# jojolebarjos/board-game-simulator-python

Measured on AMD Instinct MI355X. Metric: env-steps/sec, Connect4(6,7,4) random rollout, batch=2^20 per GPU, higher is better.
Workload: dtype u64

## Files before the change

### board-game-simulator-python_amd/csrc/bgs_host.hip

```cpp
#include <immintrin.h>
#include <limits.h>
#include <linux/futex.h>
#include <pthread.h>
#include <sched.h>
#include <sys/syscall.h>
#include <time.h>
#include <unistd.h>

#include <atomic>
#include <chrono>
#include <condition_variable>
#include <cstdlib>
#include <cstdio>
#include <algorithm>
#include <cstring>
#include <mutex>
#include <new>
#include <thread>
#include <vector>

#include "bgs_capi_util.h"
#include "bgs_common.h"
#include "bgs_internal.h"

struct bgs_event {
    int device;
    hipEvent_t ev;
};

namespace {

using bgs::fail;

struct ExpandTable {
    uint64_t pairs[256];
    ExpandTable() {
        for (int byte = 0; byte < 256; ++byte) {
            uint64_t four = 0;
            for (int j = 0; j < 4; ++j) four |= (uint64_t)bgs::reward_pair((uint32_t)(byte >> (2 * j)) & 3u) << (16 * j);
            pairs[byte] = four;
        }
    }
};
const ExpandTable g_expand;

template <bool STREAM>
__attribute__((target("avx2"))) int64_t expand_avx2(const uint8_t* src, int64_t code_bytes, int8_t* dst) {
    const __m256i spread = _mm256_setr_epi8(0, 0, 0, 0, 1, 1, 1, 1, 2, 2, 2, 2, 3, 3, 3, 3,
                                            4, 4, 4, 4, 5, 5, 5, 5, 6, 6, 6, 6, 7, 7, 7, 7);
    const __m256i field = _mm256_set1_epi32((int)0xC0300C03u);
    const __m256i one = _mm256_set1_epi32(0x40100401);
    const __m256i two = _mm256_set1_epi32((int)0x80200802u);
    int64_t i = 0;
    for (; i + 8 <= code_bytes; i += 8) {
        long long eight;
        memcpy(&eight, src + i, 8);
        const __m256i rep = _mm256_shuffle_epi8(_mm256_set1_epi64x(eight), spread);
        const __m256i f = _mm256_and_si256(rep, field);
        const __m256i is1 = _mm256_cmpeq_epi8(f, one), is2 = _mm256_cmpeq_epi8(f, two);
        const __m256i r0 = _mm256_sub_epi8(is2, is1), r1 = _mm256_sub_epi8(is1, is2);
        const __m256i lo = _mm256_unpacklo_epi8(r0, r1), hi = _mm256_unpackhi_epi8(r0, r1);
        const __m256i first = _mm256_permute2x128_si256(lo, hi, 0x20), second = _mm256_permute2x128_si256(lo, hi, 0x31);
        if (STREAM) {
            _mm256_stream_si256(reinterpret_cast<__m256i*>(dst + 8 * i), first);
            _mm256_stream_si256(reinterpret_cast<__m256i*>(dst + 8 * i + 32), second);
        } else {
            _mm256_storeu_si256(reinterpret_cast<__m256i*>(dst + 8 * i), first);
            _mm256_storeu_si256(reinterpret_cast<__m256i*>(dst + 8 * i + 32), second);
        }
    }
    if (STREAM) _mm_sfence();
    return i;
}

const bool g_have_avx2 = __builtin_cpu_supports("avx2");
const bool g_stream_stores = bgs::experiment("no_stream_stores") == nullptr;

void expand_range(const uint8_t* packed, int64_t first, int64_t count, int8_t* reward) {
    const int64_t whole = count / 4;
    const uint8_t* src = packed + first / 4;
    int8_t* out = reward + 2 * first;
    int64_t i0 = 0;
    if (g_have_avx2) {
        const bool stream = (reinterpret_cast<uintptr_t>(out) & 31u) == 0 && whole >= (1 << 14) && g_stream_stores;
        i0 = stream ? expand_avx2<true>(src, whole, out) : expand_avx2<false>(src, whole, out);
    }
    for (int64_t i = i0; i < whole; ++i) memcpy(out + 8 * i, &g_expand.pairs[src[i]], 8);
    for (int64_t g = first + whole * 4; g < first + count; ++g) {
        const uint16_t pair = bgs::reward_pair((uint32_t)(packed[g / 4] >> (2 * (g & 3))) & 3u);
        memcpy(reward + 2 * g, &pair, 2);
    }
}

struct CellFormat {
    int cells = 0;
    int nwc = 0;
    int sets = 0;
    int offset = 0;
    int weight[4] = {0, 0, 0, 0};
};

struct SpreadTable {
    uint64_t v[256];
    SpreadTable() {
        for (int byte = 0; byte < 256; ++byte) {
            uint64_t w = 0;
            for (int b = 0; b < 8; ++b) w |= (uint64_t)((byte >> b) & 1) << (8 * b);
            v[byte] = w;
        }
    }
};
const SpreadTable g_spread;

__attribute__((target("avx512f,avx512bw"))) void expand_cells_avx512(const uint64_t* wire, int64_t n, const CellFormat& f,
                                                                      int64_t first, int64_t count, int8_t* out) {
    const __m512i base = _mm512_set1_epi8((char)f.offset);
    __m512i weight[4];
    for (int p = 0; p < f.sets; ++p) weight[p] = _mm512_set1_epi8((char)f.weight[p]);
    alignas(64) int8_t block[64 * 256 + 64];
    const bool lines = f.cells <= 256 && g_stream_stores && (reinterpret_cast<uintptr_t>(out) & 63u) == 0;
#define BGS_ONE_GAME(i_)                                                                                              \
    do {                                                                                                                \
        int8_t* dst_ = out + (i_)*f.cells;                                                                              \
        for (int j = 0; j < f.nwc; ++j) {                                                                               \
            __m512i acc = base;                                                                                         \
// ... 95 lines not shown
    const bool have = fgets(list, sizeof list, f) != nullptr;
    fclose(f);
    if (!have) return false;
    cpu_set_t allowed;
    if (sched_getaffinity(0, sizeof allowed, &allowed) != 0) return false;
    int any = 0;
    char* save = nullptr;
    for (char* tok = strtok_r(list, ",\n", &save); tok; tok = strtok_r(nullptr, ",\n", &save)) {
        int lo = 0, hi = 0;
        const int k = sscanf(tok, "%d-%d", &lo, &hi);
        if (k < 1) continue;
        if (k == 1) hi = lo;
        for (int c = lo; c <= hi && c < CPU_SETSIZE; ++c)
            if (CPU_ISSET(c, &allowed)) {
                CPU_SET(c, out);
                ++any;
            }
    }
    return any > 0;
}

}

namespace {
inline bool sink_trace_on() {
    static const bool on = bgs::experiment("sink_trace") != nullptr;
    return on;
}
inline double mono_us() {
    return std::chrono::duration<double, std::micro>(std::chrono::steady_clock::now().time_since_epoch()).count();
}
}

static bool codes_hold_a_zero(const uint8_t* codes, int64_t first, int64_t count) {
    const uint8_t* p = codes + first / 4;
    const int64_t whole = count / 4;
    int64_t i = 0;
    uint64_t seen = 0;
    for (; i + 8 <= whole; i += 8) {
        uint64_t x;
        memcpy(&x, p + i, 8);
        seen |= ~(x | (x >> 1)) & 0x5555555555555555ull;
    }
    for (; i < whole; ++i) seen |= (uint64_t)(~(p[i] | (p[i] >> 1)) & 0x55u);
    for (int64_t k = 0; k < count - whole * 4; ++k) seen |= ((p[whole] >> (2 * k)) & 3u) == 0u ? 1u : 0u;
    return seen != 0;
}

struct bgs_reward_sink {
    int device = 0;
    int64_t max_games = 0;
    int slots = 0;
    int ring = 0;
    int threads = 0;
    std::vector<uint8_t*> pinned;
    std::vector<uint8_t*> mapped;
    std::vector<hipEvent_t> landed;
    bool grids = false;
    CellFormat cells;
    size_t slot_bytes = 0;
    struct Job {
        int64_t n_games = 0;
        int8_t* host_reward = nullptr;
        int event_slot = 0;
        bool all_end = false;
    };
    std::vector<Job> jobs;
    std::mutex mu;
    std::condition_variable cv_submit;
    std::condition_variable cv_landed;
    std::condition_variable cv_done;
    int64_t claimed = 0;
    int64_t submitted = 0;
    volatile int64_t* progress = nullptr;
    int64_t landed_upto = 0;
    int64_t completed = 0;
    std::vector<int> parts_done;
    std::vector<char> slot_ok;
    bool stop = false;
    std::vector<int64_t> failed_tickets;
    bool poll = false;
    std::vector<std::thread> workers;
    std::atomic<int64_t> a_submitted{0}, a_landed{0}, a_completed{0};
    std::atomic<bool> a_stop{false};
    std::atomic<int> urgent{0};
    int spin_us = 0;
    int wait_spin_us = 200;

    bool spin_for(const std::atomic<int64_t>& counter, int64_t ticket) const {
        if (counter.load(std::memory_order_acquire) > ticket) return true;
        if (spin_us <= 0) return false;
        const auto until = std::chrono::steady_clock::now() + std::chrono::microseconds(spin_us);
        for (;;) {
            for (int i = 0; i < 64; ++i) {
                if (counter.load(std::memory_order_acquire) > ticket || a_stop.load(std::memory_order_relaxed)) return true;
                _mm_pause();
            }
            if (std::chrono::steady_clock::now() >= until) return false;
        }
    }

    void work(int t) {
        (void)hipSetDevice(device);
        for (int64_t ticket = 0;; ++ticket) {
            const int slot = (int)(ticket % ring);
            Job job;
            bool ok = true;
            if (t == 0) {
                spin_for(a_submitted, ticket);
                {
                    std::unique_lock<std::mutex> lock(mu);
                    cv_submit.wait(lock, [&] { return stop || submitted > ticket; });
                    if (submitted <= ticket) return;
                    job = jobs[slot];
                }
                if (job.n_games == 0) {
                    ok = false;
                } else if (poll || urgent.load(std::memory_order_relaxed) > 0) {
                    hipError_t e;
                    while ((e = hipEventQuery(landed[job.event_slot])) == hipErrorNotReady) _mm_pause();
                    ok = e == hipSuccess;
                } else {
                    ok = hipEventSynchronize(landed[job.event_slot]) == hipSuccess;
                }
                if (sink_trace_on()) fprintf(stderr, "sink-trace ticket %lld landed %.1f\n", (long long)ticket, mono_us());
                {
                    std::lock_guard<std::mutex> lock(mu);
                    if (!ok && job.n_games != 0) failed_tickets.push_back(ticket);
                    slot_ok[slot] = ok;
                    landed_upto = ticket + 1;
                    a_landed.store(ticket + 1, std::memory_order_release);
                }
                cv_landed.notify_all();
            } else {
                if (urgent.load(std::memory_order_relaxed) > 0) {
                    const auto until = std::chrono::steady_clock::now() + std::chrono::microseconds(2000);
                    while (a_landed.load(std::memory_order_acquire) <= ticket && !a_stop.load(std::memory_order_relaxed) &&
                           urgent.load(std::memory_order_relaxed) > 0 && std::chrono::steady_clock::now() < until)
                        for (int i = 0; i < 16; ++i) _mm_pause();
                } else {
                    spin_for(a_landed, ticket);
                }
                std::unique_lock<std::mutex> lock(mu);
                cv_landed.wait(lock, [&] { return stop || landed_upto > ticket; });
                if (landed_upto <= ticket) return;
                job = jobs[slot];
                ok = slot_ok[slot];
            }
            const int expanders = threads > 1 ? threads - 1 : 1;
            const int share = threads > 1 ? t - 1 : 0;
            if (threads > 1 && t == 0) continue;
            const double trace_t0 = sink_trace_on() ? mono_us() : 0.0;
            if (ok && grids) {
                const int64_t blocks = (job.n_games + 63) / 64;
                const int64_t g0 = blocks * share / expanders * 64;
                const int64_t g1 = share + 1 == expanders ? job.n_games : blocks * (share + 1) / expanders * 64;
                static const bool skip = bgs::experiment("grid_no_expand") != nullptr;
                if (g1 > g0 && !skip) expand_cells(pinned[slot], job.n_games, cells, g0, g1 - g0, job.host_reward);
            } else if (ok) {
                const int64_t bytes = (job.n_games + 3) / 4;
                const int64_t b0 = bytes * share / expanders, b1 = bytes * (share + 1) / expanders;
                const int64_t first = b0 * 4;
                int64_t count = b1 * 4 - first;
                if (first + count > job.n_games) count = job.n_games - first;
                if (count > 0) expand_range(pinned[slot], first, count, job.host_reward);
                if (count > 0 && job.all_end && codes_hold_a_zero(pinned[slot], first, count)) {
                    std::lock_guard<std::mutex> lock(mu);
                    if (std::find(failed_tickets.begin(), failed_tickets.end(), ticket) == failed_tickets.end()) failed_tickets.push_back(ticket);
                }
            }
            if (sink_trace_on()) fprintf(stderr, "sink-trace ticket %lld worker %d expand %.1f .. %.1f\n", (long long)ticket, t, trace_t0, mono_us());
            {
                std::lock_guard<std::mutex> lock(mu);
                if (++parts_done[slot] == expanders) {
                    parts_done[slot] = 0;
                    ++completed;
                    a_completed.store(completed, std::memory_order_release);
                    cv_done.notify_all();
                    if (progress) progress_store_max(progress, completed);
                }
            }
        }
    }
};

namespace {

int64_t claim(bgs_reward_sink* s, bool ahead = false) {
    const int bound = ahead ? s->ring : s->slots;
    s->spin_for(s->a_completed, s->a_submitted.load(std::memory_order_relaxed) - bound);
    std::unique_lock<std::mutex> lock(s->mu);
    s->cv_done.wait(lock, [&] { return s->claimed - s->completed < bound; });
    return s->claimed++;
}

void publish(bgs_reward_sink* s, int64_t ticket, int64_t n_games, int8_t* host_reward, bool ok = true, int64_t event_ticket = -1,
             bool all_end = false) {
    {
        std::unique_lock<std::mutex> lock(s->mu);
// ... 147 lines not shown
    const hipError_t err = hipEventQuery(e->ev);
    if (err == hipSuccess) *done = 1;
    else if (err == hipErrorNotReady) *done = 0;
    else return fail(BGS_ERR_RUNTIME, "hipEventQuery failed: %s", hipGetErrorString(err));
    return BGS_OK;
}

int bgs_read_reward_async(bgs_batch* b, int8_t* host_dst, bgs_event* done) {
    NEED(b != nullptr && host_dst != nullptr, "NULL argument");
    int rc = enter_device(b->device);
    if (rc) return rc;
    HIP_TRY(hipMemcpyAsync(host_dst, b->d_reward, (size_t)b->n * 2, hipMemcpyDeviceToHost, b->stream));
    if (done) HIP_TRY(hipEventRecord(done->ev, b->stream));
    return BGS_OK;
}

int bgs_read_outcomes_async(bgs_batch* b, uint8_t* host_dst, bgs_event* done) {
    NEED(b != nullptr && host_dst != nullptr, "NULL argument");
    int rc = enter_device(b->device);
    if (rc) return rc;
    const size_t bytes = (size_t)(b->n + 3) / 4;
    NEED(bytes <= b->staging_bytes, "staging buffer too small");
    uint8_t* d_packed = b->d_staging;
    bgs::pack_outcomes(b, d_packed);
    HIP_TRY(hipGetLastError());
    HIP_TRY(hipMemcpyAsync(host_dst, d_packed, bytes, hipMemcpyDeviceToHost, b->stream));
    if (done) HIP_TRY(hipEventRecord(done->ev, b->stream));
    return BGS_OK;
}

int bgs_expand_outcomes_host(const uint8_t* packed, int64_t first, int64_t count, int8_t* reward) {
    NEED(packed != nullptr && reward != nullptr, "NULL argument");
    NEED(first >= 0 && count >= 0 && (first & 3) == 0, "first must be a non-negative multiple of 4, count >= 0");
    expand_range(packed, first, count, reward);
    return BGS_OK;
}

int bgs_rollout_to_host(bgs_batch* b, uint64_t seed, int32_t max_plies, uint32_t flags, void* host_dst, int codes,
                        bgs_event* done) {
    int rc = bgs_rollout(b, seed, max_plies, flags);
    if (rc) return rc;
    return codes ? bgs_read_outcomes_async(b, static_cast<uint8_t*>(host_dst), done)
                 : bgs_read_reward_async(b, static_cast<int8_t*>(host_dst), done);
}

static int make_sink(int device, int64_t max_games, int slots, int threads, size_t slot_bytes, const CellFormat* cells,
                     bgs_reward_sink** out) {
    NEED(out != nullptr, "out is NULL");
    *out = nullptr;
    NEED(max_games >= 1 && slots >= 1 && slots <= 256 && threads >= 1 && threads <= 256,
         "need max_games >= 1, 1 <= slots <= 256, 1 <= threads <= 256");
    int rc = enter_device(device);
    if (rc) return rc;
    bgs_reward_sink* s = new (std::nothrow) bgs_reward_sink();
    NEED(s != nullptr, "out of host memory");
    s->device = device;
    s->max_games = max_games;
    s->slot_bytes = slot_bytes;
    if (cells) {
        s->grids = true;
        s->cells = *cells;
    }
    s->slots = slots;
    s->ring = cells ? slots : std::max(slots, bgs::kSinkGroupRing);
    const int ring = s->ring;
    s->threads = threads;
    s->jobs.resize(ring);
    if (const char* env = bgs::experiment("sink_poll")) s->poll = atoi(env) != 0;
    if (const char* env = bgs::experiment("sink_wait_spin_us")) {
        const int v = atoi(env);
        if (v >= 0 && v <= 1000000) s->wait_spin_us = v;
    }
    if (const char* env = bgs::experiment("sink_spin_us")) {
        const int v = atoi(env);
        if (v >= 0 && v <= 1000000) s->spin_us = v;
    }
    s->parts_done.assign(ring, 0);
    s->slot_ok.assign(ring, 1);
    const size_t bytes = slot_bytes;
    hipError_t err = hipSuccess;
    const char* aff0 = getenv("BGS_SINK_AFFINITY");
    const bool place = !(aff0 && atoi(aff0) == 0);
    cpu_set_t node_cpus, caller_cpus;
    const bool moved = place && device_node_cpus(device, &node_cpus) && sched_getaffinity(0, sizeof caller_cpus, &caller_cpus) == 0 &&
                       sched_setaffinity(0, sizeof node_cpus, &node_cpus) == 0;
    for (int k = 0; k < ring && err == hipSuccess; ++k) {
        void* host = nullptr;
        void* dev = nullptr;
        hipEvent_t ev = nullptr;
        err = hipHostMalloc(&host, bytes, hipHostMallocMapped);
        if (err == hipSuccess) s->pinned.push_back(static_cast<uint8_t*>(host));
        if (err == hipSuccess) err = hipHostGetDevicePointer(&dev, host, 0);
        if (err == hipSuccess) s->mapped.push_back(static_cast<uint8_t*>(dev));
        if (err == hipSuccess) err = hipEventCreateWithFlags(&ev, hipEventDisableTiming);
        if (err == hipSuccess) s->landed.push_back(ev);
    }
    if (moved) (void)sched_setaffinity(0, sizeof caller_cpus, &caller_cpus);
// ... 254 lines not shown
```

### board-game-simulator-python_amd/csrc/connect_kernels.hip

```cpp
#include <type_traits>

#include "bgs_common.h"
#include "bgs_internal.h"
#include "connect_board.h"

#ifndef BGS_TU_ID
#define BGS_TU_ID "unknown"
#endif
extern "C" const char bgs_tu_id_connect[] = BGS_TU_ID;

namespace bgs {
namespace {

template <int NW_, int SH, int SW, int SK>
struct Geo {
    static constexpr int NW = NW_;
    static constexpr int STATIC_H = SH, STATIC_W = SW, STATIC_K = SK;
    static constexpr int MAXW = SW ? SW : BGS_CONNECT_MAX_W;
    int rh, rw, rk;
    __device__ __forceinline__ int h() const { return SH ? SH : rh; }
    __device__ __forceinline__ int w() const { return SW ? SW : rw; }
    __device__ __forceinline__ int k() const { return SK ? SK : rk; }
    __device__ __forceinline__ uint32_t all_columns() const { return (1u << w()) - 1u; }
};
// ... 632 lines not shown
            uint64_t carry;
            asm("v_mad_u64_u32 %0, %1, %2, %3, %4" : "=v"(cmp64), "=s"(carry) : "v"(idx - op), "s"(ONES), "v"(eights));
        }
        const uint32_t cmp = (uint32_t)cmp64;
        uint32_t col = (uint32_t)__popc(cmp & column_top);
        if (g.w() >= 8) col &= 7u;
        const uint32_t sh = col * 4u;
        const uint32_t v = (h4 >> sh) & 15u;
        uint32_t base = col * stride + top;
        asm("" : "+v"(base));
        uint32_t pos = base - v;
        if ((uint32_t)g.w() * stride + top > 63u) pos &= 63u;
        const uint64_t bit = 1ull << pos;
        mine = ((uint64_t)and_or((uint32_t)(bit >> 32), act, (uint32_t)(mine >> 32)) << 32) |
               and_or((uint32_t)bit, act, (uint32_t)mine);
        h4 += act << sh;
        op = (h4 >> 3) & ONES;
        if (g.k() == 4) return ply_run_of_four(g, mine, pos);
        Bits<1> b;
        b.w[0] = mine;
        return has_run(g, b);
    }
    template <uint32_t J>
    __device__ __forceinline__ void full(const G& g, uint32_t draw, uint64_t (&q)[2], uint32_t& h4, uint32_t& op,
                                         uint32_t& alive, bool& won_any) const {
        const bool won = drop(g, draw, alive, q[J & 1u], h4, op);
        won_any = won_any || won;
        alive = (won || op == 0u) ? 0u : alive;
    }
    __device__ __forceinline__ void cheap(const G& g, uint32_t j, uint32_t draw, uint64_t (&q)[2], uint32_t& h4) const {
        const uint32_t col = sample_index(draw, (uint32_t)g.w());
        const uint32_t sh = col * 4u;
        const uint32_t v = (h4 >> sh) & 15u;
        const uint32_t pos = col * stride + top - v;
        q[j & 1u] |= 1ull << pos;
        h4 -= 1u << sh;
    }
    __device__ __forceinline__ static uint32_t outcome_of(const uint64_t (&q)[2], bool won_any) {
        const uint32_t stones = (uint32_t)__popcll(q[0]) + (uint32_t)__popcll(q[1]);
        return connect_outcome_byte(stones, won_any);
    }
};

template <class G, bool CAPPED, bool FROM_INITIAL, bool CODES, bool PER_PLY>
__global__ void __launch_bounds__(BGS_BLOCK)
k_connect_rollout_aligned(G g, uint64_t* __restrict__ planes, uint8_t* __restrict__ status, uint16_t* __restrict__ reward,
                          int64_t n, uint64_t seed, uint64_t first_game, uint32_t max_plies,
                          unsigned long long* __restrict__ steps, uint32_t games_per_wave, uint32_t* __restrict__ codes_out) {
    extern __shared__ uint32_t code_lds[];
    const NibblePlies<G> plies(g);
    constexpr uint32_t ONES = NibblePlies<G>::ONES;
    const uint32_t top = plies.top, columns = plies.columns, stride = plies.stride;

    const uint32_t wave = __builtin_amdgcn_readfirstlane(blockIdx.x * (BGS_BLOCK / BGS_WAVE) + (threadIdx.x >> 6));
    const int64_t begin = (int64_t)wave * games_per_wave;
    const int64_t end = begin + games_per_wave < n ? begin + games_per_wave : n;
    const uint32_t avail = begin < end ? (uint32_t)(end - begin) : 0u;
    uint32_t taken = 0;
    uint64_t* __restrict__ const plane0 = planes + begin;
    uint64_t* __restrict__ const plane1 = planes + n + begin;
    uint8_t* __restrict__ const status_out = status + begin;
    uint16_t* __restrict__ const reward_out = reward + begin;

    uint64_t p[2] = {0, 0};
    uint32_t hts = 0;
    uint32_t blk = 0;
    uint32_t live = 0;
    uint32_t st = 0;
    uint32_t game = 0;
// ... 72 lines not shown
    } while (__builtin_amdgcn_ballot_w64(live != 0) || taken < avail);
    if (CODES) codes.flush(codes_out, begin);
    add_steps(steps, stepped);
}

template <class G, int OPEN_BLOCKS, bool PER_PLY = false>
struct OpenedWords {
    static constexpr int LAST = G::STATIC_H > 0 ? (G::STATIC_H * G::STATIC_W + 3) / 4 - 1 : 11;
    static constexpr int COUNT = PER_PLY ? 1 : (LAST - OPEN_BLOCKS + 1 > 1 ? LAST - OPEN_BLOCKS + 1 : 1);
    static constexpr int QUADS = (COUNT + 3) / 4;
    static_assert(LAST <= 11 && OPEN_BLOCKS >= 1 && OPEN_BLOCKS <= 4, "three philox calls cover blocks 0 .. 11");
};

template <int QUADS>
struct OpenedPool {
    static constexpr uint32_t SLOTS = 64;
    uint64_t plane[2][SLOTS];
    uint32_t cols[SLOTS];
    uint4 words[QUADS][SLOTS];
};

constexpr uint32_t kReplayMark = 1u << 28;
constexpr uint32_t kReplayRow = 0x80000000u;

template <class G, int OPEN_BLOCKS, bool PER_PLY>
constexpr bool deferred_opening() {
    if constexpr (G::STATIC_H > 0 && G::STATIC_W > 0 && G::STATIC_K > 0)
        return !PER_PLY && kDeferredOpeningStages > 0 && OPEN_BLOCKS == kRolloutOpeningBlocks && kRolloutOpeningBlocks == 3 &&
               deferred_opening_ok(G::STATIC_H, G::STATIC_W, G::STATIC_K);
    else
        return false;
}

template <class G, class Pool>
__device__ __forceinline__ void open_games_deferred(const G& g, Pool& pool, uint32_t slot, uint64_t seed, uint64_t id, bool mine) {
    constexpr uint32_t ONES = 0x11111111u;
    const uint32_t top = (uint32_t)g.h() + 7u;
    const uint32_t columns = ONES & ((1u << (4 * g.w())) - 1u);
    const uint32_t stride = (uint32_t)g.h() + 1u;
    uint64_t q[2] = {0, 0};
    uint32_t h4 = top * columns;
    auto cheap_ply = [&](uint32_t j, uint32_t draw, bool wrap) {
        const uint32_t col = sample_index(draw, (uint32_t)g.w());
        const uint32_t sh = col * 4u;
        const uint32_t v = (h4 >> sh) & 15u;
        uint32_t pos = col * stride + top - v;
        if (wrap) pos &= 63u;
        q[j & 1u] |= 1ull << pos;
        h4 -= 1u << sh;
    };
    auto blind_block = [&](uint32_t word, bool wrap) -> bool {
        cheap_ply(0u, sub_draw<0>(word), wrap);
        cheap_ply(1u, sub_draw<1>(word), wrap);
        cheap_ply(2u, sub_draw<2>(word), wrap);
        const bool closed = ((h4 >> 3) & ONES) != columns;
        cheap_ply(3u, sub_draw<3>(word), wrap);
        return closed;
    };
    auto park = [&](uint32_t cols, const uint4& lo, const uint4& hi) {
        pool.plane[0][slot] = q[0];
        pool.plane[1][slot] = q[1];
        pool.cols[slot] = cols;
        pool.words[0][slot] = lo;
        pool.words[1][slot] = hi;
    };
    const Philox4 a = philox4x32_10(seed, id, 0u);
    cheap_ply(0u, sub_draw<0>(a.v[0]), false);
    cheap_ply(1u, sub_draw<1>(a.v[0]), false);
    cheap_ply(2u, sub_draw<2>(a.v[0]), false);
    cheap_ply(3u, sub_draw<3>(a.v[0]), false);
    uint32_t* const slot_words0 = reinterpret_cast<uint32_t*>(&pool.words[0][slot]);
    uint32_t* const slot_words1 = reinterpret_cast<uint32_t*>(&pool.words[1][slot]);
    slot_words0[0] = a.v[1]; slot_words0[1] = a.v[2]; slot_words0[2] = a.v[3];
    uint64_t id_after = id;
    asm volatile("" : "+v"(id_after) : : "memory");
    uint32_t word9, word10;
    {
        Philox4 c = philox4x32_10(seed, id_after, 2u);
        slot_words1[3] = c.v[0];
        word9 = c.v[1];
        word10 = c.v[2];
        asm volatile("" : "+v"(id_after), "+v"(word9), "+v"(word10) : : "memory");
    }
    {
        const Philox4 b = philox4x32_10(seed, id_after, 1u);
        slot_words0[3] = b.v[0];
        slot_words1[0] = b.v[1]; slot_words1[1] = b.v[2]; slot_words1[2] = b.v[3];
    }
    pool.plane[0][slot] = q[0];
    pool.plane[1][slot] = q[1];
    pool.cols[slot] = mine ? (h4 | kReplayMark) : 0u;
    asm volatile("" ::: "memory");
    blind_block(slot_words0[0], false);
    const bool closed = blind_block(slot_words0[1], false);
    const uint32_t hits = four_in_a_row_low_hits(q[0], g.h()) | four_in_a_row_low_hits(q[1], g.h());
    const bool clean = mine && !closed && hits == 0u;
    if (clean) {
        const uint4 lo = pool.words[0][slot], hi = pool.words[1][slot];
        park(h4, make_uint4(lo.z, lo.w, hi.x, hi.y), make_uint4(hi.z, hi.w, word9, word10));
    }
    if constexpr (kDeferredOpeningStages >= 2) {
        asm volatile("" ::: "memory");
        const bool closed2 = blind_block(slot_words0[0], true);
        const uint32_t hits2 = four_in_a_row_low_hits(q[0], g.h()) | four_in_a_row_low_hits(q[1], g.h());
        if (clean && !closed2 && hits2 == 0u) {
            const uint4 lo = pool.words[0][slot], hi = pool.words[1][slot];
            park(h4, make_uint4(lo.y, lo.z, lo.w, hi.x), make_uint4(hi.y, hi.z, hi.w, 0u));
        }
    }
}

template <bool PER_PLY, uint32_t J>
__device__ __forceinline__ uint32_t opening_draw(const Philox4& own, uint32_t word) {
    return PER_PLY ? own.v[J] : sub_draw<J>(word);
}

template <int OPEN_BLOCKS, bool PER_PLY, bool BOARDS, class G, class Pool>
__device__ __forceinline__ void open_games_per_ply(const G& g, const NibblePlies<G>& plies, Pool& pool, uint64_t seed, uint64_t id,
                                                   uint32_t og, uint32_t avail, uint64_t* plane0, uint64_t* plane1, uint8_t* outcome) {
    using OW = OpenedWords<G, OPEN_BLOCKS, PER_PLY>;
    uint64_t q[2] = {0, 0};
    uint32_t h4 = plies.top * plies.columns, alive = ~0u, op = plies.columns;
    bool won_any = false;
    uint32_t words[12];
    Philox4 own = philox4x32_10(seed, id, 0u);
    if constexpr (!PER_PLY) {
        words[0] = own.v[0]; words[1] = own.v[1]; words[2] = own.v[2]; words[3] = own.v[3];
#pragma unroll
        for (int c = 1; c < 3; ++c) {
            if (4 * c <= OW::LAST) {
                const Philox4 d = philox4x32_10(seed, id, (uint32_t)c);
                words[4 * c] = d.v[0]; words[4 * c + 1] = d.v[1]; words[4 * c + 2] = d.v[2]; words[4 * c + 3] = d.v[3];
            } else {
                words[4 * c] = words[4 * c + 1] = words[4 * c + 2] = words[4 * c + 3] = 0u;
            }
        }
    } else {
#pragma unroll
        for (int c = 0; c < 12; ++c) words[c] = 0u;
    }
    plies.cheap(g, 0u, opening_draw<PER_PLY, 0>(own, words[0]), q, h4);
    plies.cheap(g, 1u, opening_draw<PER_PLY, 1>(own, words[0]), q, h4);
    plies.cheap(g, 2u, opening_draw<PER_PLY, 2>(own, words[0]), q, h4);
    plies.cheap(g, 3u, opening_draw<PER_PLY, 3>(own, words[0]), q, h4);
    if (OPEN_BLOCKS >= 2) {
        if constexpr (PER_PLY) own = philox4x32_10(seed, id, 1u);
        plies.cheap(g, 0u, opening_draw<PER_PLY, 0>(own, words[1]), q, h4);
        plies.cheap(g, 1u, opening_draw<PER_PLY, 1>(own, words[1]), q, h4);
        op = (h4 >> 3) & plies.ONES;
        plies.template full<2>(g, opening_draw<PER_PLY, 2>(own, words[1]), q, h4, op, alive, won_any);
        plies.template full<3>(g, opening_draw<PER_PLY, 3>(own, words[1]), q, h4, op, alive, won_any);
    }
#pragma unroll
    for (int ob = 2; ob < OPEN_BLOCKS; ++ob) {
        if constexpr (PER_PLY) own = philox4x32_10(seed, id, (uint32_t)ob);
        plies.template full<0>(g, opening_draw<PER_PLY, 0>(own, words[ob]), q, h4, op, alive, won_any);
        plies.template full<1>(g, opening_draw<PER_PLY, 1>(own, words[ob]), q, h4, op, alive, won_any);
        plies.template full<2>(g, opening_draw<PER_PLY, 2>(own, words[ob]), q, h4, op, alive, won_any);
        plies.template full<3>(g, opening_draw<PER_PLY, 3>(own, words[ob]), q, h4, op, alive, won_any);
    }
    if (OPEN_BLOCKS >= 2 && og < avail && alive == 0) {
        if (BOARDS || plane0) {
            plane0[og] = q[0];
            plane1[og] = q[1];
        }
        outcome[og] = (uint8_t)plies.outcome_of(q, won_any);
    }
    const uint32_t slot = og & (Pool::SLOTS - 1u);
    pool.plane[0][slot] = q[0];
    pool.plane[1][slot] = q[1];
    pool.cols[slot] = alive ? h4 : 0u;
#pragma unroll
    for (int k = 0; k < OW::QUADS; ++k) {
        auto at = [&](int i) { return OPEN_BLOCKS + i <= 11 ? words[OPEN_BLOCKS + i <= 11 ? OPEN_BLOCKS + i : 11] : 0u; };
// ... 1237 lines not shown
```

Measured before the change: 1040 billion.

## Let sink expander threads wait on events themselves and fuse zero check into expand

Removes the dedicated landing thread. Whichever expander arrives first waits on the GPU event and then advances landed_upto over every consecutive ticket that shares the same event, so all threads do expansion work. The unfinished-game check is folded into the expand pass instead of a second scan over the codes. An optional AVX-512 expand path and a configurable ring size are also added, both behind experiment flags. The aim is to cut one thread handoff and one memory pass per ticket, at the cost of more complex locking.

```diff
diff --git a/board-game-simulator-python_amd/csrc/bgs_host.hip b/board-game-simulator-python_amd/csrc/bgs_host.hip
--- a/board-game-simulator-python_amd/csrc/bgs_host.hip
+++ b/board-game-simulator-python_amd/csrc/bgs_host.hip
@@ -22,6 +22,7 @@
 #include "bgs_capi_util.h"
 #include "bgs_common.h"
 #include "bgs_internal.h"
+#include "sink_expand.h"
 
 struct bgs_event {
     int device;
@@ -32,65 +33,21 @@
 
 using bgs::fail;
 
-struct ExpandTable {
-    uint64_t pairs[256];
-    ExpandTable() {
-        for (int byte = 0; byte < 256; ++byte) {
-            uint64_t four = 0;
-            for (int j = 0; j < 4; ++j) four |= (uint64_t)bgs::reward_pair((uint32_t)(byte >> (2 * j)) & 3u) << (16 * j);
-            pairs[byte] = four;
-        }
-    }
-};
-const ExpandTable g_expand;
-
-template <bool STREAM>
-__attribute__((target("avx2"))) int64_t expand_avx2(const uint8_t* src, int64_t code_bytes, int8_t* dst) {
-    const __m256i spread = _mm256_setr_epi8(0, 0, 0, 0, 1, 1, 1, 1, 2, 2, 2, 2, 3, 3, 3, 3,
-                                            4, 4, 4, 4, 5, 5, 5, 5, 6, 6, 6, 6, 7, 7, 7, 7);
-    const __m256i field = _mm256_set1_epi32((int)0xC0300C03u);
-    const __m256i one = _mm256_set1_epi32(0x40100401);
-    const __m256i two = _mm256_set1_epi32((int)0x80200802u);
-    int64_t i = 0;
-    for (; i + 8 <= code_bytes; i += 8) {
-        long long eight;
-        memcpy(&eight, src + i, 8);
-        const __m256i rep = _mm256_shuffle_epi8(_mm256_set1_epi64x(eight), spread);
-        const __m256i f = _mm256_and_si256(rep, field);
-        const __m256i is1 = _mm256_cmpeq_epi8(f, one), is2 = _mm256_cmpeq_epi8(f, two);
-        const __m256i r0 = _mm256_sub_epi8(is2, is1), r1 = _mm256_sub_epi8(is1, is2);
-        const __m256i lo = _mm256_unpacklo_epi8(r0, r1), hi = _mm256_unpackhi_epi8(r0, r1);
-        const __m256i first = _mm256_permute2x128_si256(lo, hi, 0x20), second = _mm256_permute2x128_si256(lo, hi, 0x31);
-        if (STREAM) {
-            _mm256_stream_si256(reinterpret_cast<__m256i*>(dst + 8 * i), first);
-            _mm256_stream_si256(reinterpret_cast<__m256i*>(dst + 8 * i + 32), second);
-        } else {
-            _mm256_storeu_si256(reinterpret_cast<__m256i*>(dst + 8 * i), first);
-            _mm256_storeu_si256(reinterpret_cast<__m256i*>(dst + 8 * i + 32), second);
-        }
-    }
-    if (STREAM) _mm_sfence();
-    return i;
-}
-
-const bool g_have_avx2 = __builtin_cpu_supports("avx2");
 const bool g_stream_stores = bgs::experiment("no_stream_stores") == nullptr;
 
-void expand_range(const uint8_t* packed, int64_t first, int64_t count, int8_t* reward) {
-    const int64_t whole = count / 4;
-    const uint8_t* src = packed + first / 4;
-    int8_t* out = reward + 2 * first;
-    int64_t i0 = 0;
-    if (g_have_avx2) {
-        const bool stream = (reinterpret_cast<uintptr_t>(out) & 31u) == 0 && whole >= (1 << 14) && g_stream_stores;
-        i0 = stream ? expand_avx2<true>(src, whole, out) : expand_avx2<false>(src, whole, out);
-    }
-    for (int64_t i = i0; i < whole; ++i) memcpy(out + 8 * i, &g_expand.pairs[src[i]], 8);
-    for (int64_t g = first + whole * 4; g < first + count; ++g) {
-        const uint16_t pair = bgs::reward_pair((uint32_t)(packed[g / 4] >> (2 * (g & 3))) & 3u);
-        memcpy(reward + 2 * g, &pair, 2);
-    }
-}
+#ifdef BGS_TEST_HOOKS
+int expand_form() {
+    const char* e = bgs::experiment("sink_expand");
+    if (e == nullptr) return bgs::kSinkExpandAuto;
+    const int form = strcmp(e, "table") == 0 ? bgs::kSinkExpandTable : strcmp(e, "avx2") == 0 ? bgs::kSinkExpandAvx2 :
+                     strcmp(e, "avx512") == 0 ? bgs::kSinkExpandAvx512 : -1;
+    return form > 0 && bgs::sink_expand_has(form) ? form : -1;
+}
+#define BGS_NEED_EXPAND_FORM(form_) NEED((form_) >= 0, "experiment sink_expand: table, avx2 or avx512, and only a form this CPU has")
+#else
+constexpr int expand_form() { return bgs::kSinkExpandAuto; }
+#define BGS_NEED_EXPAND_FORM(form_) (void)(form_)
+#endif
 
 struct CellFormat {
     int cells = 0;
@@ -252,21 +209,6 @@
 }
 }
 
-static bool codes_hold_a_zero(const uint8_t* codes, int64_t first, int64_t count) {
-    const uint8_t* p = codes + first / 4;
-    const int64_t whole = count / 4;
-    int64_t i = 0;
-    uint64_t seen = 0;
-    for (; i + 8 <= whole; i += 8) {
-        uint64_t x;
-        memcpy(&x, p + i, 8);
-        seen |= ~(x | (x >> 1)) & 0x5555555555555555ull;
-    }
-    for (; i < whole; ++i) seen |= (uint64_t)(~(p[i] | (p[i] >> 1)) & 0x55u);
-    for (int64_t k = 0; k < count - whole * 4; ++k) seen |= ((p[whole] >> (2 * k)) & 3u) == 0u ? 1u : 0u;
-    return seen != 0;
-}
-
 struct bgs_reward_sink {
     int device = 0;
     int64_t max_games = 0;
@@ -297,12 +239,14 @@
     int64_t completed = 0;
     std::vector<int> parts_done;
     std::vector<char> slot_ok;
+    bool waiting = false;
+    int expand_form = 0;
     bool stop = false;
     std::vector<int64_t> failed_tickets;
     bool poll = false;
     std::vector<std::thread> workers;
     std::atomic<int64_t> a_submitted{0}, a_landed{0}, a_completed{0};
-    std::atomic<bool> a_stop{false};
+    std::atomic<bool> a_stop{false}, a_waiting{false};
     std::atomic<int> urgent{0};
     int spin_us = 0;
     int wait_spin_us = 200;
@@ -320,20 +264,29 @@
         }
     }
 
-    void work(int t) {
-        (void)hipSetDevice(device);
-        for (int64_t ticket = 0;; ++ticket) {
-            const int slot = (int)(ticket % ring);
-            Job job;
-            bool ok = true;
-            if (t == 0) {
-                spin_for(a_submitted, ticket);
-                {
-                    std::unique_lock<std::mutex> lock(mu);
-                    cv_submit.wait(lock, [&] { return stop || submitted > ticket; });
-                    if (submitted <= ticket) return;
-                    job = jobs[slot];
+    bool await_landed(int64_t ticket) {
+        spin_for(a_landed, ticket);
+        if (a_landed.load(std::memory_order_acquire) > ticket) return true;
+        bool may_spin = true;
+        std::unique_lock<std::mutex> lock(mu);
+        for (;;) {
+            if (landed_upto > ticket) return true;
+            if (stop && submitted <= landed_upto) return false;
+            if (!waiting) {
+                waiting = true;
+                a_waiting.store(true, std::memory_order_relaxed);
+                const int64_t w = landed_upto;
+                cv_submit.wait(lock, [&] { return stop || submitted > w; });
+                if (submitted <= w) {
+                    waiting = false;
+                    a_waiting.store(false, std::memory_order_relaxed);
+                    lock.unlock();
+                    cv_landed.notify_all();
+                    return false;
                 }
+                const Job job = jobs[w % ring];
+                lock.unlock();
+                bool ok = true;
                 if (job.n_games == 0) {
                     ok = false;
                 } else if (poll || urgent.load(std::memory_order_relaxed) > 0) {
@@ -343,33 +296,49 @@
                 } else {
                     ok = hipEventSynchronize(landed[job.event_slot]) == hipSuccess;
                 }
-                if (sink_trace_on()) fprintf(stderr, "sink-trace ticket %lld landed %.1f\n", (long long)ticket, mono_us());
-                {
-                    std::lock_guard<std::mutex> lock(mu);
-                    if (!ok && job.n_games != 0) failed_tickets.push_back(ticket);
-                    slot_ok[slot] = ok;
-                    landed_upto = ticket + 1;
-                    a_landed.store(ticket + 1, std::memory_order_release);
+                const double trace_t = sink_trace_on() ? mono_us() : 0.0;
+                lock.lock();
+                int64_t upto = w;
+                for (;;) {
+                    if (!ok && job.n_games != 0) failed_tickets.push_back(upto);
+                    slot_ok[upto % ring] = ok;
+                    ++upto;
+                    if (job.n_games == 0 || upto >= submitted) break;
+                    const Job& next = jobs[upto % ring];
+                    if (next.n_games == 0 || next.event_slot != job.event_slot) break;
                 }
+                landed_upto = upto;
+                a_landed.store(upto, std::memory_order_release);
+                waiting = false;
+                a_waiting.store(false, std::memory_order_relaxed);
                 cv_landed.notify_all();
-            } else {
-                if (urgent.load(std::memory_order_relaxed) > 0) {
-                    const auto until = std::chrono::steady_clock::now() + std::chrono::microseconds(2000);
-                    while (a_landed.load(std::memory_order_acquire) <= ticket && !a_stop.load(std::memory_order_relaxed) &&
-                           urgent.load(std::memory_order_relaxed) > 0 && std::chrono::steady_clock::now() < until)
-                        for (int i = 0; i < 16; ++i) _mm_pause();
-                } else {
-                    spin_for(a_landed, ticket);
-                }
-                std::unique_lock<std::mutex> lock(mu);
-                cv_landed.wait(lock, [&] { return stop || landed_upto > ticket; });
-                if (landed_upto <= ticket) return;
-                job = jobs[slot];
-                ok = slot_ok[slot];
-            }
-            const int expanders = threads > 1 ? threads - 1 : 1;
-            const int share = threads > 1 ? t - 1 : 0;
-            if (threads > 1 && t == 0) continue;
+                if (sink_trace_on())
+                    for (int64_t k = w; k < upto; ++k) fprintf(stderr, "sink-trace ticket %lld landed %.1f\n", (long long)k, trace_t);
+                continue;
+            }
+            if (may_spin && urgent.load(std::memory_order_relaxed) > 0) {
+                lock.unlock();
+                const auto until = std::chrono::steady_clock::now() + std::chrono::microseconds(2000);
+                while (a_landed.load(std::memory_order_acquire) <= ticket && a_waiting.load(std::memory_order_relaxed) &&
+                       !a_stop.load(std::memory_order_relaxed) && urgent.load(std::memory_order_relaxed) > 0 &&
+                       std::chrono::steady_clock::now() < until)
+                    for (int i = 0; i < 16; ++i) _mm_pause();
+                may_spin = false;
+                lock.lock();
+                continue;
+            }
+            cv_landed.wait(lock, [&] { return stop || landed_upto > ticket || !waiting; });
+        }
+    }
+
+    void work(int t) {
+        (void)hipSetDevice(device);
+        for (int64_t ticket = 0;; ++ticket) {
+            const int slot = (int)(ticket % ring);
+            if (!await_landed(ticket)) return;
+            const Job job = jobs[slot];
+            const bool ok = slot_ok[slot] != 0;
+            const int expanders = threads, share = t;
             const double trace_t0 = sink_trace_on() ? mono_us() : 0.0;
             if (ok && grids) {
                 const int64_t blocks = (job.n_games + 63) / 64;
@@ -383,8 +352,7 @@
                 const int64_t first = b0 * 4;
                 int64_t count = b1 * 4 - first;
                 if (first + count > job.n_games) count = job.n_games - first;
-                if (count > 0) expand_range(pinned[slot], first, count, job.host_reward);
-                if (count > 0 && job.all_end && codes_hold_a_zero(pinned[slot], first, count)) {
+                if (count > 0 && bgs::sink_expand(pinned[slot], first, count, job.host_reward, expand_form, g_stream_stores) && job.all_end) {
                     std::lock_guard<std::mutex> lock(mu);
                     if (std::find(failed_tickets.begin(), failed_tickets.end(), ticket) == failed_tickets.end()) failed_tickets.push_back(ticket);
                 }
@@ -598,7 +566,9 @@
 int bgs_expand_outcomes_host(const uint8_t* packed, int64_t first, int64_t count, int8_t* reward) {
     NEED(packed != nullptr && reward != nullptr, "NULL argument");
     NEED(first >= 0 && count >= 0 && (first & 3) == 0, "first must be a non-negative multiple of 4, count >= 0");
-    expand_range(packed, first, count, reward);
+    const int form = expand_form();
+    BGS_NEED_EXPAND_FORM(form);
+    (void)bgs::sink_expand(packed, first, count, reward, form, g_stream_stores);
     return BGS_OK;
 }
 
@@ -616,11 +586,14 @@
     *out = nullptr;
     NEED(max_games >= 1 && slots >= 1 && slots <= 256 && threads >= 1 && threads <= 256,
          "need max_games >= 1, 1 <= slots <= 256, 1 <= threads <= 256");
+    const int form = expand_form();
+    BGS_NEED_EXPAND_FORM(form);
     int rc = enter_device(device);
     if (rc) return rc;
     bgs_reward_sink* s = new (std::nothrow) bgs_reward_sink();
     NEED(s != nullptr, "out of host memory");
     s->device = device;
+    s->expand_form = form;
     s->max_games = max_games;
     s->slot_bytes = slot_bytes;
     if (cells) {
@@ -628,7 +601,12 @@
         s->cells = *cells;
     }
     s->slots = slots;
-    s->ring = cells ? slots : std::max(slots, bgs::kSinkGroupRing);
+    int group_ring = bgs::kSinkGroupRing;
+    if (const char* env = bgs::experiment("sink_ring")) {
+        const int v = atoi(env);
+        if (v >= 1 && v <= 256) group_ring = v;
+    }
+    s->ring = cells ? slots : std::max(slots, group_ring);
     const int ring = s->ring;
     s->threads = threads;
     s->jobs.resize(ring);
diff --git a/board-game-simulator-python_amd/csrc/sink_expand.h b/board-game-simulator-python_amd/csrc/sink_expand.h
--- /dev/null
+++ b/board-game-simulator-python_amd/csrc/sink_expand.h
@@ -0,0 +1,136 @@
+#pragma once
+#include <immintrin.h>
+#include <stdint.h>
+#include <string.h>
+
+namespace bgs {
+
+enum SinkExpandForm { kSinkExpandAuto = 0, kSinkExpandTable = 1, kSinkExpandAvx2 = 2, kSinkExpandAvx512 = 3 };
+
+namespace sink_expand_detail {
+
+constexpr uint16_t pair_of(uint32_t code) { return code == 1u ? (uint16_t)0xFF01u : code == 2u ? (uint16_t)0x01FFu : (uint16_t)0u; }
+
+struct Table {
+    uint64_t pairs[256];
+    Table() {
+        for (int byte = 0; byte < 256; ++byte) {
+            uint64_t four = 0;
+            for (int j = 0; j < 4; ++j) four |= (uint64_t)pair_of((uint32_t)(byte >> (2 * j)) & 3u) << (16 * j);
+            pairs[byte] = four;
+        }
+    }
+};
+inline const Table& table() {
+    static const Table t;
+    return t;
+}
+
+inline uint64_t zero_fields(uint64_t x) { return ~(x | (x >> 1)) & 0x5555555555555555ull; }
+
+inline uint64_t expand_table(const uint8_t* src, int64_t n, int8_t* dst) {
+    const Table& t = table();
+    uint64_t seen = 0;
+    for (int64_t i = 0; i < n; ++i) {
+        memcpy(dst + 8 * i, &t.pairs[src[i]], 8);
+        seen |= zero_fields(src[i]) & 0x55u;
+    }
+    return seen;
+}
+
+template <bool STREAM>
+__attribute__((target("avx2"))) inline int64_t expand_avx2(const uint8_t* src, int64_t code_bytes, int8_t* dst, uint64_t* seen) {
+    const __m256i spread = _mm256_setr_epi8(0, 0, 0, 0, 1, 1, 1, 1, 2, 2, 2, 2, 3, 3, 3, 3,
+                                            4, 4, 4, 4, 5, 5, 5, 5, 6, 6, 6, 6, 7, 7, 7, 7);
+    const __m256i field = _mm256_set1_epi32((int)0xC0300C03u);
+    const __m256i one = _mm256_set1_epi32(0x40100401);
+    const __m256i two = _mm256_set1_epi32((int)0x80200802u);
+    uint64_t zeros = 0;
+    int64_t i = 0;
+    for (; i + 8 <= code_bytes; i += 8) {
+        long long eight;
+        memcpy(&eight, src + i, 8);
+        zeros |= zero_fields((uint64_t)eight);
+        const __m256i rep = _mm256_shuffle_epi8(_mm256_set1_epi64x(eight), spread);
+        const __m256i f = _mm256_and_si256(rep, field);
+        const __m256i is1 = _mm256_cmpeq_epi8(f, one), is2 = _mm256_cmpeq_epi8(f, two);
+        const __m256i r0 = _mm256_sub_epi8(is2, is1), r1 = _mm256_sub_epi8(is1, is2);
+        const __m256i lo = _mm256_unpacklo_epi8(r0, r1), hi = _mm256_unpackhi_epi8(r0, r1);
+        const __m256i first = _mm256_permute2x128_si256(lo, hi, 0x20), second = _mm256_permute2x128_si256(lo, hi, 0x31);
+        if (STREAM) {
+            _mm256_stream_si256(reinterpret_cast<__m256i*>(dst + 8 * i), first);
+            _mm256_stream_si256(reinterpret_cast<__m256i*>(dst + 8 * i + 32), second);
+        } else {
+            _mm256_storeu_si256(reinterpret_cast<__m256i*>(dst + 8 * i), first);
+            _mm256_storeu_si256(reinterpret_cast<__m256i*>(dst + 8 * i + 32), second);
+        }
+    }
+    if (STREAM) _mm_sfence();
+    *seen |= zeros;
+    return i;
+}
+
+template <bool STREAM>
+__attribute__((target("avx512f,avx512bw"))) inline int64_t expand_avx512(const uint8_t* src, int64_t code_bytes, int8_t* dst, uint64_t* seen) {
+    const __m512i spread = _mm512_set_epi64(0x0707070707070707ll, 0x0606060606060606ll, 0x0505050505050505ll, 0x0404040404040404ll,
+                                            0x0303030303030303ll, 0x0202020202020202ll, 0x0101010101010101ll, 0x0000000000000000ll);
+    const __m512i field = _mm512_set1_epi64((long long)0xC0C030300C0C0303ull);
+    const __m512i one = _mm512_set1_epi64(0x4040101004040101ll);
+    const __m512i two = _mm512_set1_epi64((long long)0x8080202008080202ull);
+    const __m512i first_wins = _mm512_set1_epi16((short)0xFF01);
+    const __m512i second_wins = _mm512_set1_epi16((short)0x01FF);
+    uint64_t zeros = 0;
+    int64_t i = 0;
+    for (; i + 8 <= code_bytes; i += 8) {
+        long long eight;
+        memcpy(&eight, src + i, 8);
+        zeros |= zero_fields((uint64_t)eight);
+        const __m512i f = _mm512_and_si512(_mm512_shuffle_epi8(_mm512_set1_epi64(eight), spread), field);
+        const __mmask64 is1 = _mm512_cmpeq_epi8_mask(f, one), is2 = _mm512_cmpeq_epi8_mask(f, two);
+        const __m512i line = _mm512_mask_mov_epi8(_mm512_maskz_mov_epi8(is1, first_wins), is2, second_wins);
+        if (STREAM) _mm512_stream_si512(reinterpret_cast<__m512i*>(dst + 8 * i), line);
+        else _mm512_storeu_si512(dst + 8 * i, line);
+    }
+    if (STREAM) _mm_sfence();
+    *seen |= zeros;
+    return i;
+}
+
+}
+
+inline bool sink_expand_has(int form) {
+    static const bool avx2 = __builtin_cpu_supports("avx2");
+    static const bool avx512 = __builtin_cpu_supports("avx512f") && __builtin_cpu_supports("avx512bw");
+    return form == kSinkExpandAvx2 ? avx2 : form == kSinkExpandAvx512 ? avx512 : true;
+}
+
+inline int sink_expand_best() { return sink_expand_has(kSinkExpandAvx2) ? kSinkExpandAvx2 : kSinkExpandTable; }
+
+inline bool sink_expand(const uint8_t* packed, int64_t first, int64_t count, int8_t* reward, int form = kSinkExpandAuto,
+                        bool stream = true) {
+    using namespace sink_expand_detail;
+    if (form == kSinkExpandAuto) form = sink_expand_best();
+    const int64_t whole = count / 4;
+    const uint8_t* src = packed + first / 4;
+    int8_t* out = reward + 2 * first;
+    uint64_t seen = 0;
+    int64_t i = 0;
+    if (form != kSinkExpandTable && whole >= 8) {
+        const uintptr_t store = form == kSinkExpandAvx512 ? 63u : 31u;
+        const bool streams = stream && (reinterpret_cast<uintptr_t>(out) & store) == 0 && whole >= (1 << 14);
+        if (form == kSinkExpandAvx512)
+            i += streams ? expand_avx512<true>(src + i, whole - i, out + 8 * i, &seen) : expand_avx512<false>(src + i, whole - i, out + 8 * i, &seen);
+        else
+            i += streams ? expand_avx2<true>(src + i, whole - i, out + 8 * i, &seen) : expand_avx2<false>(src + i, whole - i, out + 8 * i, &seen);
+    }
+    seen |= expand_table(src + i, whole - i, out + 8 * i);
+    for (int64_t g = first + whole * 4; g < first + count; ++g) {
+        const uint32_t code = (uint32_t)(packed[g / 4] >> (2 * (g & 3))) & 3u;
+        const uint16_t pair = pair_of(code);
+        memcpy(reward + 2 * g, &pair, 2);
+        seen |= code == 0u ? 1u : 0u;
+    }
+    return seen != 0;
+}
+
+}
```

After: 1039 billion. About the same (-0.0%).

## Share Philox first-round work across counter blocks and slim opening-pool LDS traffic

Applied to the files above, without the earlier changes.

Adds a Philox variant that computes the first-round product on the game id once and reuses it for all three counter blocks of a game. Specializes the first opening ply to write the board and height state directly instead of a generic read-modify-write. Replaces the 128-bit word reloads and re-parks in the deferred opening with 64-bit volatile LDS moves that shift only the words that need shifting. Adds compiler barriers on the position base to steer instruction selection. The aim is fewer ALU cycles in RNG and opening setup and less LDS traffic, at the cost of more register pressure and hand-written volatile LDS accesses that could break if the pool layout changes.

```diff
diff --git a/board-game-simulator-python_amd/csrc/connect_kernels.hip b/board-game-simulator-python_amd/csrc/connect_kernels.hip
--- a/board-game-simulator-python_amd/csrc/connect_kernels.hip
+++ b/board-game-simulator-python_amd/csrc/connect_kernels.hip
@@ -688,9 +688,21 @@
         const uint32_t col = sample_index(draw, (uint32_t)g.w());
         const uint32_t sh = col * 4u;
         const uint32_t v = (h4 >> sh) & 15u;
-        const uint32_t pos = col * stride + top - v;
+        uint32_t base = col * stride + top;
+        asm("" : "+v"(base));
+        const uint32_t pos = base - v;
         q[j & 1u] |= 1ull << pos;
         h4 -= 1u << sh;
+    }
+    __device__ __forceinline__ void cheap_first(const G& g, uint32_t draw, uint64_t (&q)[2], uint32_t& h4) const {
+        if constexpr (G::STATIC_H <= 0) {
+            cheap(g, 0u, draw, q, h4);
+            return;
+        }
+        const uint32_t col = sample_index(draw, (uint32_t)g.w());
+        q[0] = 1ull << (col * stride);
+        q[1] = 0;
+        h4 = top * columns - (1u << (col * 4u));
     }
     __device__ __forceinline__ static uint32_t outcome_of(const uint64_t (&q)[2], bool won_any) {
         const uint32_t stones = (uint32_t)__popcll(q[0]) + (uint32_t)__popcll(q[1]);
@@ -829,6 +841,54 @@
         return false;
 }
 
+struct PhiloxShared {
+    uint32_t c3;
+    uint64_t p1;
+};
+__device__ __forceinline__ PhiloxShared philox_shared(uint64_t seed, uint64_t game) {
+    const uint64_t p0 = (uint64_t)0xD2511F53u * (uint32_t)game;
+    const uint32_t n2 = xor3((uint32_t)(p0 >> 32), 0u, (uint32_t)(seed >> 32));
+    PhiloxShared s;
+    s.c3 = (uint32_t)p0;
+    s.p1 = (uint64_t)0xCD9E8D57u * n2;
+    return s;
+}
+__device__ __forceinline__ Philox4 philox_shared_10(const PhiloxShared& s, uint64_t seed, uint64_t game, uint32_t block) {
+    uint32_t k0 = (uint32_t)seed, k1 = (uint32_t)(seed >> 32);
+    const uint64_t q1 = (uint64_t)0xCD9E8D57u * block;
+    uint32_t c0 = xor3((uint32_t)(q1 >> 32), (uint32_t)(game >> 32), k0);
+    uint32_t c1 = (uint32_t)q1, c2, c3;
+    k0 += 0x9E3779B9u;
+    k1 += 0xBB67AE85u;
+    {
+        const uint64_t p0 = (uint64_t)0xD2511F53u * c0;
+        const uint32_t n0 = xor3((uint32_t)(s.p1 >> 32), c1, k0);
+        const uint32_t n2 = xor3((uint32_t)(p0 >> 32), s.c3, k1);
+        c1 = (uint32_t)s.p1;
+        c3 = (uint32_t)p0;
+        c0 = n0;
+        c2 = n2;
+        k0 += 0x9E3779B9u;
+        k1 += 0xBB67AE85u;
+    }
+#pragma unroll
+    for (int r = 2; r < 10; ++r) {
+        const uint64_t p0 = (uint64_t)0xD2511F53u * c0;
+        const uint64_t p1 = (uint64_t)0xCD9E8D57u * c2;
+        const uint32_t n0 = xor3((uint32_t)(p1 >> 32), c1, k0);
+        const uint32_t n2 = xor3((uint32_t)(p0 >> 32), c3, k1);
+        c1 = (uint32_t)p1;
+        c3 = (uint32_t)p0;
+        c0 = n0;
+        c2 = n2;
+        k0 += 0x9E3779B9u;
+        k1 += 0xBB67AE85u;
+    }
+    Philox4 out;
+    out.v[0] = c0; out.v[1] = c1; out.v[2] = c2; out.v[3] = c3;
+    return out;
+}
+
 template <class G, class Pool>
 __device__ __forceinline__ void open_games_deferred(const G& g, Pool& pool, uint32_t slot, uint64_t seed, uint64_t id, bool mine) {
     constexpr uint32_t ONES = 0x11111111u;
@@ -841,7 +901,9 @@
         const uint32_t col = sample_index(draw, (uint32_t)g.w());
         const uint32_t sh = col * 4u;
         const uint32_t v = (h4 >> sh) & 15u;
-        uint32_t pos = col * stride + top - v;
+        uint32_t base = col * stride + top;
+        asm("" : "+v"(base));
+        uint32_t pos = base - v;
         if (wrap) pos &= 63u;
         q[j & 1u] |= 1ull << pos;
         h4 -= 1u << sh;
@@ -854,55 +916,73 @@
         cheap_ply(3u, sub_draw<3>(word), wrap);
         return closed;
     };
-    auto park = [&](uint32_t cols, const uint4& lo, const uint4& hi) {
+    auto park = [&](uint32_t cols) {
         pool.plane[0][slot] = q[0];
         pool.plane[1][slot] = q[1];
         pool.cols[slot] = cols;
-        pool.words[0][slot] = lo;
-        pool.words[1][slot] = hi;
     };
-    const Philox4 a = philox4x32_10(seed, id, 0u);
-    cheap_ply(0u, sub_draw<0>(a.v[0]), false);
+    PhiloxShared shared = philox_shared(seed, id);
+    const Philox4 a = philox_shared_10(shared, seed, id, 0u);
+    {
+        const uint32_t col = sample_index(sub_draw<0>(a.v[0]), (uint32_t)g.w());
+        q[0] = 1ull << (col * stride);
+        h4 -= 1u << (col * 4u);
+    }
     cheap_ply(1u, sub_draw<1>(a.v[0]), false);
     cheap_ply(2u, sub_draw<2>(a.v[0]), false);
     cheap_ply(3u, sub_draw<3>(a.v[0]), false);
-    uint32_t* const slot_words0 = reinterpret_cast<uint32_t*>(&pool.words[0][slot]);
-    uint32_t* const slot_words1 = reinterpret_cast<uint32_t*>(&pool.words[1][slot]);
+    typedef volatile __attribute__((address_space(3))) uint32_t LdsWord;
+    typedef volatile __attribute__((address_space(3))) uint64_t LdsPair;
+    LdsWord* const slot_words0 = (LdsWord*)&pool.words[0][slot];
+    LdsWord* const slot_words1 = (LdsWord*)&pool.words[1][slot];
+    LdsPair* const slot_pairs0 = (LdsPair*)&pool.words[0][slot];
+    LdsPair* const slot_pairs1 = (LdsPair*)&pool.words[1][slot];
     slot_words0[0] = a.v[1]; slot_words0[1] = a.v[2]; slot_words0[2] = a.v[3];
     uint64_t id_after = id;
-    asm volatile("" : "+v"(id_after) : : "memory");
-    uint32_t word9, word10;
+    asm volatile("" : "+v"(id_after), "+v"(shared.c3), "+v"(shared.p1) : : "memory");
+    uint64_t words9_10;
     {
-        Philox4 c = philox4x32_10(seed, id_after, 2u);
+        Philox4 c = philox_shared_10(shared, seed, id_after, 2u);
         slot_words1[3] = c.v[0];
-        word9 = c.v[1];
-        word10 = c.v[2];
-        asm volatile("" : "+v"(id_after), "+v"(word9), "+v"(word10) : : "memory");
+        words9_10 = ((uint64_t)c.v[2] << 32) | c.v[1];
+        asm volatile("" : "+v"(id_after), "+v"(words9_10), "+v"(shared.c3), "+v"(shared.p1) : : "memory");
     }
     {
-        const Philox4 b = philox4x32_10(seed, id_after, 1u);
+        const Philox4 b = philox_shared_10(shared, seed, id_after, 1u);
         slot_words0[3] = b.v[0];
         slot_words1[0] = b.v[1]; slot_words1[1] = b.v[2]; slot_words1[2] = b.v[3];
     }
-    pool.plane[0][slot] = q[0];
-    pool.plane[1][slot] = q[1];
-    pool.cols[slot] = mine ? (h4 | kReplayMark) : 0u;
+    park(mine ? (h4 | kReplayMark) : 0u);
     asm volatile("" ::: "memory");
-    blind_block(slot_words0[0], false);
-    const bool closed = blind_block(slot_words0[1], false);
+    const uint64_t words1_2 = slot_pairs0[0];
+    blind_block((uint32_t)words1_2, false);
+    const bool closed = blind_block((uint32_t)(words1_2 >> 32), false);
     const uint32_t hits = four_in_a_row_low_hits(q[0], g.h()) | four_in_a_row_low_hits(q[1], g.h());
     const bool clean = mine && !closed && hits == 0u;
     if (clean) {
-        const uint4 lo = pool.words[0][slot], hi = pool.words[1][slot];
-        park(h4, make_uint4(lo.z, lo.w, hi.x, hi.y), make_uint4(hi.z, hi.w, word9, word10));
+        const uint64_t words3_4 = slot_pairs0[1], words5_6 = slot_pairs1[0], words7_8 = slot_pairs1[1];
+        park(h4);
+        slot_pairs0[0] = words3_4;
+        slot_pairs0[1] = words5_6;
+        slot_pairs1[0] = words7_8;
+        slot_pairs1[1] = words9_10;
     }
     if constexpr (kDeferredOpeningStages >= 2) {
         asm volatile("" ::: "memory");
         const bool closed2 = blind_block(slot_words0[0], true);
         const uint32_t hits2 = four_in_a_row_low_hits(q[0], g.h()) | four_in_a_row_low_hits(q[1], g.h());
         if (clean && !closed2 && hits2 == 0u) {
-            const uint4 lo = pool.words[0][slot], hi = pool.words[1][slot];
-            park(h4, make_uint4(lo.y, lo.z, lo.w, hi.x), make_uint4(hi.y, hi.z, hi.w, 0u));
+            const uint32_t word4 = slot_words0[1];
+            const uint64_t words5_6 = slot_pairs0[1], words7_8 = slot_pairs1[0], words9_10_back = slot_pairs1[1];
+            park(h4);
+            slot_words0[0] = word4;
+            slot_words0[1] = (uint32_t)words5_6;
+            slot_words0[2] = (uint32_t)(words5_6 >> 32);
+            slot_words0[3] = (uint32_t)words7_8;
+            slot_words1[0] = (uint32_t)(words7_8 >> 32);
+            slot_words1[1] = (uint32_t)words9_10_back;
+            slot_words1[2] = (uint32_t)(words9_10_back >> 32);
+            slot_words1[3] = 0u;
         }
     }
 }
@@ -936,7 +1016,7 @@
 #pragma unroll
         for (int c = 0; c < 12; ++c) words[c] = 0u;
     }
-    plies.cheap(g, 0u, opening_draw<PER_PLY, 0>(own, words[0]), q, h4);
+    plies.cheap_first(g, opening_draw<PER_PLY, 0>(own, words[0]), q, h4);
     plies.cheap(g, 1u, opening_draw<PER_PLY, 1>(own, words[0]), q, h4);
     plies.cheap(g, 2u, opening_draw<PER_PLY, 2>(own, words[0]), q, h4);
     plies.cheap(g, 3u, opening_draw<PER_PLY, 3>(own, words[0]), q, h4);
```

Result: faster. 1041 billion before, 1067 billion after, median of 6 (+2.5%).
